# domkirke/acids_transforms

Hardware: AMD Instinct MI355X
Metric: spectrogram frames/sec (fwd+invert), n_fft=1024 hop=256 (higher is better)
Workload: dtype f32; 1 GPU; configs[1]: batch=1024 clips/GPU x 4 s mono 44.1 kHz, STFT fwd + Magnitude(mel=128, log1p, unipolar) [one fused kernel] + ISTFT invert, fp32; n_fft=1024, hop=256, frames_per_clip=690, clips_per_gpu=1024

## Files before the change

### acids_transforms_amd/csrc/fft512.h

```cpp
#pragma once
#include <hip/hip_runtime.h>
#include <stdint.h>

#include "fastmath.h"
#include "inv1024_pairs.h"

namespace at_hip {

#ifndef AT_WAVE_PRIORITY
#define AT_WAVE_PRIORITY 1
#endif
template <int LEVEL>
__device__ __forceinline__ void wave_priority() {
#if AT_WAVE_PRIORITY
  __builtin_amdgcn_s_setprio(LEVEL);
#endif
}

constexpr int kFftLdsFloat2PerWave = 568;

constexpr int kTwiddleCount = 22 * 64;
constexpr int kTileCtrSlots = 4096;

__device__ __forceinline__ float2 cadd(float2 a, float2 b) { return make_float2(a.x + b.x, a.y + b.y); }

typedef float v2f __attribute__((ext_vector_type(2)));

__device__ __forceinline__ v2f to_v(float2 a) { return (v2f){a.x, a.y}; }
// ... 110 lines not shown
  __device__ __forceinline__ v2f getr(int m) const { return tr[m]; }
  __device__ __forceinline__ v2f getr_self() const { return tr_self; }
};

template <bool INV>
struct LdsTwiddles {
  const float2* tab;
  int lane;
  __device__ __forceinline__ v2f get1(int k) const { return lds_read_single(reinterpret_cast<const v2f*>(tab) + k * 64 + lane); }
  __device__ __forceinline__ v2f get2(int k) const { return lds_read_single(reinterpret_cast<const v2f*>(tab) + (7 + k) * 64 + lane); }
  __device__ __forceinline__ v2f getr(int m) const { return lds_read_single(reinterpret_cast<const v2f*>(tab) + (14 + m) * 64 + lane); }
  __device__ __forceinline__ v2f getr_self() const { return lds_read_single(reinterpret_cast<const v2f*>(tab) + (14 + inv1024::kSelfPairedRow) * 64); }
};
struct HybridTwiddles {
  v2f t1[7];
  v2f t2[7];
  const float2* tab;
  int col;
  __device__ __forceinline__ v2f get1(int k) const { return t1[k]; }
  __device__ __forceinline__ v2f get2(int k) const { return t2[k]; }
  __device__ __forceinline__ v2f getr(int m) const { return lds_read_single(reinterpret_cast<const v2f*>(tab) + (14 + m) * 64 + col); }
};

template <bool INV>
__device__ __forceinline__ float2 twiddle_for_lds(const float2* __restrict__ tab, int i) {
  const float2 a = tab[i];
  return (!INV && i >= 14 * 64) ? make_float2(0.5f * a.x, 0.5f * a.y) : a;
}

template <bool INV>
__device__ __forceinline__ void load_twiddles(Twiddles& tw, const float2* __restrict__ tab, int lane) {
#pragma unroll
  for (int k = 0; k < 7; ++k) {
    tw.t1[k] = to_v(tab[k * 64 + lane]);
    tw.t2[k] = to_v(tab[(7 + k) * 64 + lane]);
  }
#pragma unroll
  for (int m = 0; m < 8; ++m) tw.tr[m] = to_v(twiddle_for_lds<INV>(tab, (14 + m) * 64 + lane));
  if (INV) {
    const float2 w = tab[(14 + inv1024::kSelfPairedRow) * 64];
    tw.tr_self = (v2f){__int_as_float(__builtin_amdgcn_readfirstlane(__float_as_int(w.x))),
                       __int_as_float(__builtin_amdgcn_readfirstlane(__float_as_int(w.y)))};
  }
}

#ifndef AT_XCHG1_SWAP
// ... 17 lines not shown
        const auto sw = __builtin_amdgcn_permlane16_swap(__float_as_uint(v[k][c]), __float_as_uint(v[k + 2][c]), false, false);
        v[k][c] = __uint_as_float(sw[0]);
        v[k + 2][c] = __uint_as_float(sw[1]);
      }
#pragma unroll
  for (int k = 0; k < 8; k += 2)
#pragma unroll
    for (int c = 0; c < 2; ++c) {
      const int a = __float_as_int(v[k][c]), b = __float_as_int(v[k + 1][c]);
      const int a2 = __builtin_amdgcn_update_dpp(a, b, 0x128, 0xf, 0xc, false);
      const int b2 = __builtin_amdgcn_update_dpp(b, a, 0x128, 0xf, 0x3, false);
      v[k][c] = __int_as_float(a2);
      v[k + 1][c] = __int_as_float(b2);
    }
}

template <bool INV, typename TW>
__device__ __forceinline__ void fft512(v2f (&v)[8], const TW& tw, float2* lds_f2, int lane, int out_lane = -1) {
  if (out_lane < 0) out_lane = lane;
  v2f* lds = reinterpret_cast<v2f*>(lds_f2);
  const int lo = lane & 7, hi = lane >> 3;
  radix8<INV>(v);
#pragma unroll
  for (int k = 1; k < 8; ++k) v[k] = twiddle<INV>(v[k], tw.get1(k - 1));
  if constexpr (AT_XCHG1_SWAP == 2 || (AT_XCHG1_SWAP == 1 && !INV)) {
    xchg1_registers(v);
  } else {
#pragma unroll
    for (int k = 0; k < 8; ++k) lds[hi * 72 + lo + 8 * k] = v[k];
    wave_lds_sync();
#pragma unroll
    for (int k = 0; k < 8; ++k) v[k] = lds_read_single(lds + k * 72 + lane);
    wave_lds_sync();
  }
  radix8<INV>(v);
#pragma unroll
  for (int k = 1; k < 8; ++k) v[k] = twiddle<INV>(v[k], tw.get2(k - 1));
#pragma unroll
  for (int k = 0; k < 8; ++k) lds[lo * 66 + hi + 8 * k] = v[k];
  wave_lds_sync();
#pragma unroll
  for (int k = 0; k < 8; ++k) v[k] = lds_read_single(lds + k * 66 + out_lane);
  wave_lds_sync();
  radix8<INV>(v);
}
constexpr bool fft512_exchanges_cover(int lo_slot, int hi_slot) {
  for (int s = lo_slot; s <= hi_slot; ++s) {
    bool hit = false;
    for (int a = 0; a < 8 && !hit; ++a) {
      if (s >= a * 72 && s < a * 72 + 64) hit = true;
      if (s >= a * 66 && s < a * 66 + 64) hit = true;
    }
    if (!hit) return false;
  }
  return true;
}
static_assert(AT_XCHG1_SWAP || (fft512_exchanges_cover(256, 319) && 320 <= kFftLdsFloat2PerWave),
              "the fixed-length mel epilogue reads absrow[513..639] uncleared: both exchanges must rewrite float2 slots 256..319");

template <bool INV, typename TW>
// ... 53 lines not shown
template <int Q, int WS>
__device__ __forceinline__ void irfft_presplit(const v2f (&x)[Q], float nyq_re, int lane, const v2f* w, v2f (&z)[Q]) {
  v2f v[Q], pm[Q];
#pragma unroll
  for (int m = 0; m < Q; ++m) v[m] = x[m];
  if (lane == 0) v[0].y = 0.0f;
  mirror_regs<Q>(v, pm, lane);
  if (lane == 0) pm[0] = (v2f){nyq_re, 0.0f};
#pragma unroll
  for (int m = 0; m < Q; ++m) {
    const v2f e = add_conj(v[m], pm[m]);
    const v2f d = cmul_conj_v(sub_conj(v[m], pm[m]), w[WS * m]);
    z[m] = add_pi(e, d);
  }
}

template <typename TW>
__device__ __forceinline__ void rfft_merge(v2f (&v)[8], const TW& tw, int lane, float2& nyq) {
  const v2f hh = {0.5f, 0.5f};
  v2f p[8];
  mirror_regs<8>(v, p, lane);
  nyq = make_float2(v[0].x - v[0].y, 0.0f);
#pragma unroll
  for (int m = 0; m < 8; ++m) {
    const v2f e = add_conj(v[m], p[m]);
    const v2f d = sub_conj(v[m], p[m]);
    const v2f wd = cmul_v(d, tw.getr(m));
    v[m] = scale_add_mi(e, hh, wd);
  }
}
template <typename TW>
__device__ __forceinline__ void rfft_merge_rot(v2f (&v)[8], const TW& tw, int lane, int rot, int col, float2& nyq) {
  const v2f hh = {0.5f, 0.5f};
  v2f p[8];
  mirror_regs_rot<8>(v, p, lane, rot, col);
  nyq = make_float2(v[0].x - v[0].y, 0.0f);
#pragma unroll
  for (int m = 0; m < 8; ++m) {
    const v2f e = add_conj(v[m], p[m]);
    const v2f d = sub_conj(v[m], p[m]);
    const v2f wd = cmul_v(d, tw.getr(m));
    v[m] = scale_add_mi(e, hh, wd);
  }
}
template <typename TW>
__device__ __forceinline__ void rfft_merge(float2 (&f)[8], const TW& tw, int lane, float2& nyq) {
  v2f v[8];
#pragma unroll
  for (int m = 0; m < 8; ++m) v[m] = to_v(f[m]);
  rfft_merge(v, tw, lane, nyq);
#pragma unroll
  for (int m = 0; m < 8; ++m) f[m] = to_f2(v[m]);
}

template <typename TW>
__device__ __forceinline__ void irfft_split(v2f (&v)[8], const TW& tw, int lane, v2f x256) {
  if (lane == 0) {
    v[0].y = 0.0f;
    v[7].y = 0.0f;
  }
#pragma unroll
  for (int m = 0; m < inv1024::kPairs; ++m) {
    const int n = inv1024::partner_reg(m);
    const v2f e = add_conj(v[m], v[n]);
    const v2f d = cmul_conj_v(sub_conj(v[m], v[n]), tw.getr(m));
// ... 63 lines not shown
```

### acids_transforms_amd/csrc/stft1024.hip

```cpp
#include <hip/hip_runtime.h>
#include "fastmath.h"
#include <type_traits>
#include <stdint.h>
#include <stdlib.h>
#include <stdio.h>
#include <string.h>
#include <atomic>

#include "band_bank.h"
#include "fft512.h"
#include "fwd1024_forms.h"
#include "run_plan.h"
#include "stft_launch.h"
#include "variants.h"

#ifndef AT_ISTFT_NT
#define AT_ISTFT_NT 1
#endif
#ifndef AT_ISTFT_NTLOAD
#define AT_ISTFT_NTLOAD 1
#endif

namespace at_hip {

constexpr int N = 1024;
constexpr int F = 513;
constexpr int WAVES_PER_BLOCK = 4;

struct FwdParams {
  const float* x;
  const float* window;
  const float2* tw;
  float2* out;
  float* phase;
  long long B, L, clip_stride, T;
  long long total_frames;
  long long frames_per_block;
  int hop;
  int center;
};

__device__ __forceinline__ void load_frame(const FwdParams& p, long long f, int lane, float2 (&v)[8]) {
  const long long b = f / p.T;
// ... 97 lines not shown
__device__ __forceinline__ float2 load_pair(const float* clip, long long L, long long i0, bool interior, bool aligned,
                                            int lane_off) {
  if (interior) {
    if (aligned) return reinterpret_cast<const float2*>(clip + i0)[lane_off >> 1];
    return make_float2(clip[i0 + lane_off], clip[i0 + lane_off + 1]);
  }
  return make_float2(clip[reflect_index(i0 + lane_off, L)], clip[reflect_index(i0 + lane_off + 1, L)]);
}


__device__ __forceinline__ float fwd_contrast(float v, int mode, float eps) { return band_contrast_fast(v, mode, eps); }

template <class Form>
__global__ __launch_bounds__(64 * Form::waves, fwd1024::waves_per_simd<Form>()) void stft1024_h256_fwd_kernel(FwdRunParams p) {
  constexpr bool WRITE_PHASE = Form::write_phase, TWLDS = Form::lds_twiddles, POLAR = Form::polar;
  constexpr bool AL = Form::aligned_stores, NT = Form::nontemporal, FP2 = Form::fixed_power2, PW = Form::persistent;
  constexpr int MEL = Form::mel, FWD_WAVES = Form::waves, CMBUF = Form::window_passes, HS = Form::hop_slots;
  constexpr int SP = Form::hoisted_passes, FQ0 = Form::fixed_quads0, FQ1 = Form::fixed_quads1, FC = Form::fixed_contrast;
  constexpr int HYB = Form::register_tables, FNP = Form::packed_passes;
  constexpr fqp_t FQP = Form::packed_quads;
  constexpr int H = 128 * HS;
  constexpr int kNP = FQP ? FNP : 1;
  constexpr int kPkStride = (kNP + 3) / 4 * 4;
  constexpr int kTabTw = TWLDS ? kTwiddleCount : 0;
  constexpr int kFeatCarry = FQP ? 128 : 0;
  constexpr int kWaveLds = kFftLdsFloat2PerWave + kFeatCarry;
  __shared__ float2 lds_all[FWD_WAVES * kWaveLds + kTabTw + 512];
  extern __shared__ float4 band_lds[];
  const int lane = threadIdx.x & 63;
  const int wave = __builtin_amdgcn_readfirstlane(threadIdx.x >> 6);
  float2* lds = lds_all + wave * kWaveLds + kFeatCarry;
  float2* tab = lds_all + FWD_WAVES * kWaveLds;
  float2 raw_first[8];
  auto load_first_frame = [&](const long long run, float2 (&raw)[8]) {
    const long long b = run / p.runs_per_clip;
    if (b >= p.B) return;
    const long long t0 = (run - b * p.runs_per_clip) * p.frames_per_run;
    if (t0 >= p.T) return;
    const float* clip = p.x + b * p.clip_stride;
    const bool clip_aligned = ((((uintptr_t)clip) & 7) == 0);
    const long long s0 = t0 * (128 * HS) - 512;
#pragma unroll
    for (int m = 0; m < 8; ++m) {
      const long long i0 = s0 + 128 * m;
      raw[m] = load_pair(clip, p.L, i0, i0 >= 0 && i0 + 128 <= p.L, clip_aligned, 2 * lane);
    }
  };
  if constexpr (!PW) load_first_frame((long long)blockIdx.x * FWD_WAVES + wave, raw_first);
  if (TWLDS)
    for (int i = threadIdx.x; i < kTwiddleCount; i += 64 * FWD_WAVES) tab[i] = twiddle_for_lds<false>(p.tw, i);
  for (int i = threadIdx.x; i < 512; i += 64 * FWD_WAVES)
    tab[kTabTw + i] = reinterpret_cast<const float2*>(p.window)[i];
  float* wlds = reinterpret_cast<float*>(band_lds);
  int* lane_tab = nullptr;
  if (MEL != 0) {
    int table_floats = 0;
    for (int q = 0; q < p.bank.n_passes; ++q) table_floats += 64 * p.bank.pass_len[q];
    for (int i = threadIdx.x; i < table_floats; i += 64 * FWD_WAVES) wlds[i] = p.bank.weights[i];
    lane_tab = reinterpret_cast<int*>(wlds + table_floats);
    for (int i = threadIdx.x; i < 64 * p.bank.n_passes; i += 64 * FWD_WAVES) {
      lane_tab[i] = p.bank.lane_start[i];
      lane_tab[64 * p.bank.n_passes + i] = p.bank.lane_filter[i];
    }
    if constexpr (FQP != 0) {
      int* pk_tab = lane_tab + 2 * 64 * p.bank.n_passes;
      for (int i = threadIdx.x; i < 64 * kNP; i += 64 * FWD_WAVES) {
        const int q = i >> 6, l = i & 63;
        const int f = p.bank.lane_filter[i];
        pk_tab[l * kPkStride + q] = (p.bank.lane_start[i] * 4) | ((f >= 0 ? f * 4 : 0xfff) << 12);
      }
    }
  }
  __shared__ unsigned s_tile[2];
  if (PW && threadIdx.x == 0) s_tile[0] = atomicAdd(p.tile_ctr, 1u);
#if AT_XCHG1_SWAP
  if (MEL != 0) {
    reinterpret_cast<float*>(lds)[512 + lane] = 0.0f;
    reinterpret_cast<float*>(lds)[576 + lane] = 0.0f;
  }
#endif
  __syncthreads();

  int sp_f[SP > 0 ? SP : 1], sp_start[SP > 0 ? SP : 1], sp_quads[SP > 0 ? SP : 1];
  if constexpr (SP > 0) {
#pragma unroll
    for (int q = 0; q < SP; ++q) {
      sp_f[q] = lane_tab[(SP + q) * 64 + lane];
      sp_start[q] = lane_tab[q * 64 + lane];
      sp_quads[q] = p.bank.pass_len[q] >> 2;
    }
  }
  Twiddles tw_regs;
  if (!TWLDS) load_twiddles<false>(tw_regs, p.tw, lane);
  const LdsTwiddles<false> tw_lds = {tab, lane};
  HybridTwiddles tw_hyb;
  if constexpr (TWLDS && (HYB & 1)) {
#pragma unroll
    for (int k = 0; k < 7; ++k) {
      tw_hyb.t1[k] = to_v(p.tw[k * 64 + lane]);
      tw_hyb.t2[k] = to_v(p.tw[(7 + k) * 64 + lane]);
    }
    tw_hyb.tab = tab;
    tw_hyb.col = lane;
  }
  const float2* win = tab + kTabTw;
  v2f win_regs[8];
  if constexpr ((HYB & 2) != 0) {
#pragma unroll
    for (int m = 0; m < 8; ++m) win_regs[m] = to_v(reinterpret_cast<const float2*>(p.window)[lane + 64 * m]);
  }

  const long long L = p.L;
  const int lane2 = 2 * lane;

  auto do_run = [&](const long long run, const bool preloaded) {
  const long long b = run / p.runs_per_clip;
  if (b >= p.B) return;
  const long long r = run - b * p.runs_per_clip;
// ... 47 lines not shown
  };
  long long t_cur = t0;
  float cm[CMBUF ? CMBUF : 1][8];
  int cm_held[CMBUF ? CMBUF : 1];
#pragma unroll
  for (int q = 0; q < (CMBUF ? CMBUF : 1); ++q) {
    cm_held[q] = 0;
#pragma unroll
    for (int k = 0; k < 8; ++k) cm[q][k] = 0.f;
  }
  float mel_off = 0.f, mel_inv = 1.f;
  if (MEL != 0 && p.offset) {
    mel_off = *p.offset;
    mel_inv = 1.0f / *p.scale;
  }

  float2 nyq_pending = make_float2(0.f, 0.f);
  float2* nyq_dst = nullptr;
  auto flush_nyquist = [&]() {
    if (nyq_dst != nullptr && lane == 0) *nyq_dst = nyq_pending;
    if (WRITE_PHASE && nyq_dst != nullptr && lane == 0)
      p.phase[(nyq_dst - p.out)] = fast_atan2f(nyq_pending.y, nyq_pending.x);
  };
  auto frame_body = [&](const float2 (&fresh)[HS]) {
    wave_priority<3>();
    float2 v[8];
#pragma unroll
    for (int m = 0; m < 8; ++m) {
      const v2f w = (HYB & 2) ? win_regs[m] : lds_read_single(reinterpret_cast<const v2f*>(win) + lane + 64 * m);
      v[m] = make_float2(raw[m].x * w.x, raw[m].y * w.y);
    }
#pragma unroll
    for (int m = 0; m < 8 - HS; ++m) raw[m] = raw[m + HS];
#pragma unroll
    for (int k = 0; k < HS; ++k) raw[8 - HS + k] = fresh[k];
    float2 nyq;
    const int col = AL ? ((lane - rot) & 63) : lane;
    {
      v2f z[8];
#pragma unroll
      for (int m = 0; m < 8; ++m) z[m] = to_v(v[m]);
      if constexpr (AL && (HYB & 1)) {
        fft512<false>(z, tw_hyb, lds, lane, col);
        tw_hyb.col = col;
        rfft_merge_rot(z, tw_hyb, lane, rot, col, nyq);
      } else if constexpr (AL) {
        fft512<false>(z, tw_lds, lds, lane, col);
        const LdsTwiddles<false> tw_col = {tab, col};
        rfft_merge_rot(z, tw_col, lane, rot, col, nyq);
      } else if constexpr (TWLDS && (HYB & 1)) {
        fft512<false>(z, tw_hyb, lds, lane);
        rfft_merge(z, tw_hyb, lane, nyq);
      } else if (TWLDS) {
        fft512<false>(z, tw_lds, lds, lane);
        rfft_merge(z, tw_lds, lane, nyq);
      } else {
        fft512<false>(z, tw_regs, lds, lane);
        rfft_merge(z, tw_regs, lane, nyq);
      }
#pragma unroll
      for (int m = 0; m < 8; ++m) v[m] = to_f2(z[m]);
      if constexpr (AL) {
        wave_priority<1>();
        const bool lo = lane < rot;
        const v2f s0 = lo ? carry : z[0];
        if (head) {
          if (!lo) put(sp, s0);
          head = false;
        } else {
          put(sp, s0);
        }
// ... 205 lines not shown
        one_pass(0, std::integral_constant<int, 0>());
        if constexpr (CMBUF >= 2) one_pass(1, std::integral_constant<int, 1>());
      } else if constexpr (SP >= 1) {
        one_pass(0, std::integral_constant<int, -1>());
        if constexpr (SP >= 2) one_pass(1, std::integral_constant<int, -1>());
      } else {
        for (int q = 0; q < p.bank.n_passes; ++q) one_pass(q, std::integral_constant<int, -1>());
      }
      wave_lds_sync();
      frow += feat_ld;
      ++t_cur;
    }
    nyq_pending = nyq;
    nyq_dst = (MEL != 2 && !AL) ? row + 512 : nullptr;
    row += F;
  };

  long long t = t0;
  long long t_fast_end = (L >= 512) ? (L - 512) / H : 0;
  if (t_fast_end > t1) t_fast_end = t1;
  if (!clip_aligned) t_fast_end = t0;
  if (t < t_fast_end) {
    const float2* nsrc = reinterpret_cast<const float2*>(clip + t * H + 512) + lane;
    for (; t < t_fast_end; ++t) {
      flush_nyquist();
      float2 fresh[HS];
#pragma unroll
      for (int k = 0; k < HS; ++k) fresh[k] = nsrc[64 * k];
      nsrc += H / 2;
      frame_body(fresh);
    }
  }
  for (; t < t1; ++t) {
    flush_nyquist();
    float2 fresh[HS];
#pragma unroll
    for (int k = 0; k < HS; ++k) fresh[k] = make_float2(0.f, 0.f);
    if (t + 1 < t1) {
#pragma unroll
      for (int k = 0; k < HS; ++k) {
        const long long i0 = t * H + 512 + 128 * k;
        fresh[k] = load_pair(clip, L, i0, i0 >= 0 && i0 + 128 <= L, clip_aligned, lane2);
      }
    }
    frame_body(fresh);
  }
  flush_nyquist();
  if constexpr (AL) {
    if (lane < rot) put(sp, carry);
  }
  if constexpr (FQP != 0) {
    wave_lds_sync();
    const float* fbuf = reinterpret_cast<const float*>(lds) - 2 * kFeatCarry;
    const float4 v = reinterpret_cast<const float4*>(fbuf)[lane];
    const float vv[4] = {v.x, v.y, v.z, v.w};
#pragma unroll
    for (int c = 0; c < 4; ++c)
      if (4 * lane + c < fc && 4 * lane + c >= fhead) fdst[4 * lane + c] = vv[c];
    wave_lds_sync();
  }
  };

  if constexpr (!PW) {
    do_run((long long)blockIdx.x * FWD_WAVES + wave, true);
  } else {
    for (int it = 0;; ++it) {
      const unsigned tile = __builtin_amdgcn_readfirstlane(s_tile[it & 1]);
      if (tile >= p.n_tiles) break;
// ... 123 lines not shown
  x256 = gl_update(q.rmid, q.tmid, q.amid, mom);
}

template <int IN_MODE>
__device__ __forceinline__ void load_spectrum(const InvParams& p, long long f, int lane, float2 (&v)[8], float2& x256) {
  RawFrame<IN_MODE> q;
  load_raw(p, f, lane, q);
  raw_to_spectrum(q, v, x256);
}

__device__ __forceinline__ float2 scaled_window(const float* window, int i) {
  const float2 w = reinterpret_cast<const float2*>(window)[i];
  return make_float2(w.x * (1.0f / 1024.0f), w.y * (1.0f / 1024.0f));
}

template <typename TW>
__device__ __forceinline__ void synth_frame_nowin(const float2 (&v)[8], float2 x256, const TW& tw, float2* lds, int lane,
                                                  v2f (&z)[8]) {
#pragma unroll
  for (int m = 0; m < 8; ++m) z[m] = to_v(v[m]);
  irfft_split(z, tw, lane, to_v(x256));
  fft512<true>(z, tw, lds, lane);
}
__device__ __forceinline__ v2f ola_window(const float2* win, int lane, int m) {
  return lds_read_single(reinterpret_cast<const v2f*>(win) + lane + 64 * m);
}

template <typename TW>
__device__ __forceinline__ void synth_frame(float2 (&v)[8], float2 x256, const TW& tw, const float2* win,
                                            float2* lds, int lane) {
  v2f z[8];
#pragma unroll
  for (int m = 0; m < 8; ++m) z[m] = to_v(v[m]);
  irfft_split(z, tw, lane, to_v(x256));
  fft512<true>(z, tw, lds, lane);
#pragma unroll
  for (int m = 0; m < 8; ++m) {
    const v2f w = lds_read_single(reinterpret_cast<const v2f*>(win) + lane + 64 * m);
    v[m] = to_f2(z[m] * w);
  }
}

template <int IN_MODE, int DEPTH, bool TWLDS, int HS = 2>
__global__ __launch_bounds__(64 * WAVES_PER_BLOCK, IN_MODE == IN_GL ? 2 : (TWLDS ? 5 : 4) - DEPTH) void istft1024_ola_kernel(InvParams p) {
  constexpr int R = 8 / HS;
  constexpr int C = 4 / HS;
  constexpr int H = 128 * HS;
  constexpr int kFull = (1 << R) - 1;
  __shared__ float2 lds_all[WAVES_PER_BLOCK * kFftLdsFloat2PerWave + 512 + (TWLDS ? kTwiddleCount : 0)];
  const int lane = threadIdx.x & 63;
  const int wave = __builtin_amdgcn_readfirstlane(threadIdx.x >> 6);
  float2* lds = lds_all + wave * kFftLdsFloat2PerWave;
  float2* win = lds_all + WAVES_PER_BLOCK * kFftLdsFloat2PerWave;
  float2* twtab = win + 512;
  for (int i = threadIdx.x; i < 512; i += 64 * WAVES_PER_BLOCK) win[i] = scaled_window(p.window, i);
  if (TWLDS)
    for (int i = threadIdx.x; i < kTwiddleCount; i += 64 * WAVES_PER_BLOCK) twtab[i] = p.tw[i];
  __syncthreads();

  const long long run = (long long)blockIdx.x * WAVES_PER_BLOCK + wave;
  const long long b = run / p.runs_per_clip;
  if (b >= p.B) return;
  const long long r = run - b * p.runs_per_clip;
  const long long nslots = p.T - 1;
  const long long j0 = r * p.slots_per_run;
  long long j1 = j0 + p.slots_per_run;
  if (j1 > nslots) j1 = nslots;
  if (j0 >= j1) return;

  Twiddles tw_regs;
  if (!TWLDS) load_twiddles<true>(tw_regs, p.tw, lane);
  const LdsTwiddles<true> tw_lds = {twtab, lane};
  auto synth = [&](const float2 (&v)[8], float2 x256, v2f (&z)[8]) {
    if (TWLDS) synth_frame_nowin(v, x256, tw_lds, lds, lane, z);
    else synth_frame_nowin(v, x256, tw_regs, lds, lane, z);
  };

  v2f acc[8];
#pragma unroll
  for (int m = 0; m < 8; ++m) acc[m] = (v2f){0.f, 0.f};

  const long long fbase = b * p.T;
  float* yclip = p.y + b * (H * nslots);
  long long t = (j0 + C - (R - 1) > 0) ? j0 + C - (R - 1) : 0;
  const long long t_last = j1 - 1 + C;
  const long long t_have = (t_last < p.T - 1) ? t_last : p.T - 1;

  RawFrame<IN_MODE> q0 = {}, q1 = {};
  if (t <= t_have) load_raw(p, fbase + t, lane, q0);
  if (t + 1 <= t_have) load_raw(p, fbase + t + 1, lane, q1);

  auto consume = [&](const RawFrame<IN_MODE>& q) {
    float2 v[8];
    float2 x256;
    if constexpr (IN_MODE == IN_GL) raw_to_spectrum(q, v, x256, p.gl_mom);
    else raw_to_spectrum(q, v, x256);
    v2f z[8];
    synth(v, x256, z);
#pragma unroll
    for (int m = 0; m < 8; ++m) acc[m] = __builtin_elementwise_fma(z[m], ola_window(win, lane, m), acc[m]);
  };
  auto put_y = [&](float2* dst, float2 val) {
#if AT_ISTFT_NT
    __builtin_nontemporal_store((v2f){val.x, val.y}, reinterpret_cast<v2f*>(dst));
#else
    *dst = val;
#endif
  };
  static_assert(sizeof(v2f) == sizeof(float2), "");
  auto emit = [&](long long j, const float2* env) {
    float2* dst = reinterpret_cast<float2*>(yclip + j * H);
#pragma unroll
    for (int k = 0; k < HS; ++k) {
      const float2 e = env[lane + 64 * k];
      put_y(dst + lane + 64 * k, make_float2(acc[k].x / e.x, acc[k].y / e.y));
    }
  };
  float2 rcp[HS];
  auto emit_fast = [&](long long j) {
    float2* dst = reinterpret_cast<float2*>(yclip + j * H);
#pragma unroll
    for (int k = 0; k < HS; ++k) put_y(dst + lane + 64 * k, make_float2(acc[k].x * rcp[k].x, acc[k].y * rcp[k].y));
  };
// ... 26 lines not shown
        const long long tt = t - (R - 1) + q;
        if (tt >= 0 && tt < p.T) mask |= 1 << q;
      }
      if (mask == kFull) emit_fast(j);
      else emit(j, reinterpret_cast<const float2*>(p.env + mask * H));
    }
    advance();
    ++t;
  };

  long long fast_begin = j0 + C > R - 1 ? j0 + C : R - 1;
  long long fast_end = (j1 - 1 + C < t_have - 2) ? j1 - 1 + C : t_have - 2;
  while (t < fast_begin && t <= t_last) generic_step();
  if (t <= fast_end) {
    if (DEPTH == 2) {
      auto fast_step = [&](RawFrame<IN_MODE>& q) {
        const RawFrame<IN_MODE> cur = q;
        load_raw(p, fbase + t + 2, lane, q);
        consume(cur);
        emit_fast(t - C);
        advance();
        ++t;
      };
      while (t + 1 <= fast_end) {
        fast_step(q0);
        fast_step(q1);
      }
    } else {
      q1 = {};
      for (; t <= fast_end; ++t) {
        const RawFrame<IN_MODE> cur = q0;
        load_raw(p, fbase + t + 1, lane, q0);
        consume(cur);
        emit_fast(t - C);
        advance();
      }
      q1 = {};
      if (t + 1 <= t_have) load_raw(p, fbase + t + 1, lane, q1);
    }
  }
  while (t <= t_last) generic_step();
}

template <int IN_MODE, int NW, int OCC>
__global__ __launch_bounds__(64 * NW, OCC) void istft1024_tile_kernel(InvParams p) {
  constexpr int HS = 2, R = 4, H = 256;
  constexpr int kFull = (1 << R) - 1;
  static_assert(IN_MODE != IN_GL, "the Griffin-Lim form keeps the long-run kernel");
  __shared__ float2 lds_all[NW * kFftLdsFloat2PerWave + 512];
  __shared__ float4 park_all[NW * 6 * 64];
  const int lane = threadIdx.x & 63;
  const int wave = __builtin_amdgcn_readfirstlane(threadIdx.x >> 6);
  float2* lds = lds_all + wave * kFftLdsFloat2PerWave;
  float2* win = lds_all + NW * kFftLdsFloat2PerWave;

  const long long tile = blockIdx.x;
  const long long b = tile / p.runs_per_clip;
  const long long k = tile - b * p.runs_per_clip;
  const long long n = p.slots_per_run;
  const long long T = p.T;
  const long long tile0 = k * p.frames_per_block;
  long long tile1 = tile0 + p.frames_per_block;
  if (tile1 > T) tile1 = T;
  auto share = [&](int w, long long& a, long long& e) {
    a = tile0 + w * n;
    if (a > tile1) a = tile1;
    e = (w == NW - 1) ? tile1 : a + n;
    if (e > tile1) e = tile1;
  };
  long long ta, tb;
  share(wave, ta, tb);
  bool self_cool = true;
  if (wave < NW - 1) {
    long long a2, e2;
    share(wave + 1, a2, e2);
    self_cool = e2 - a2 < 3;
  }
  long long t_stop = (self_cool && tb > ta) ? tb + 3 : tb;
  if (t_stop > T) t_stop = T;
  const bool parks = wave > 0 && ta > 0;
  const long long pe0 = ta == 0 ? 2 : ta + 3;
  const long long pe1 = tb + 3;

  const long long fbase = b * T;
  float* yclip = p.y + b * (H * (T - 1));
  long long t = ta;
  RawFrame<IN_MODE> q0 = {}, q1 = {};
  if (t < t_stop) load_raw(p, fbase + t, lane, q0);
  if (t + 1 < t_stop) load_raw(p, fbase + t + 1, lane, q1);

  for (int i = threadIdx.x; i < 512; i += 64 * NW) win[i] = scaled_window(p.window, i);
  Twiddles tw;
  load_twiddles<true>(tw, p.tw, lane);
  __syncthreads();

  v2f acc[8];
#pragma unroll
  for (int m = 0; m < 8; ++m) acc[m] = (v2f){0.f, 0.f};
  auto consume = [&](const RawFrame<IN_MODE>& q, v2f (&z)[8]) {
    float2 v[8];
    float2 x256;
    raw_to_spectrum(q, v, x256);
    synth_frame_nowin(v, x256, tw, lds, lane, z);
#pragma unroll
    for (int m = 0; m < 8; ++m) acc[m] = __builtin_elementwise_fma(z[m], ola_window(win, lane, m), acc[m]);
  };
  auto put_y = [&](float2* dst, float2 val) {
    __builtin_nontemporal_store((v2f){val.x, val.y}, reinterpret_cast<v2f*>(dst));
  };
  float2 rcp[HS];
  {
    const float2* env_full = reinterpret_cast<const float2*>(p.env + kFull * H);
#pragma unroll
    for (int kk = 0; kk < HS; ++kk) {
      const float2 e = env_full[lane + 64 * kk];
      rcp[kk] = make_float2(1.0f / e.x, 1.0f / e.y);
    }
  }
  auto emit_regs = [&](long long hp, v2f a0, v2f a1) {
    float2* dst = reinterpret_cast<float2*>(yclip + (hp - 2) * H);
    if (hp >= 3 && hp < T) {
      put_y(dst + lane, make_float2(a0.x * rcp[0].x, a0.y * rcp[0].y));
      put_y(dst + lane + 64, make_float2(a1.x * rcp[1].x, a1.y * rcp[1].y));
    } else {
      int mask = 0;
#pragma unroll
      for (int q = 0; q < R; ++q) {
        const long long tt = hp - (R - 1) + q;
// ... 27 lines not shown
    }
    if (t >= pe0 && t < pe1) emit_regs(t, acc[0], acc[1]);
    advance();
    ++t;
  };

  long long fast_begin = ta + 3 > pe0 ? ta + 3 : pe0;
  if (fast_begin < 3) fast_begin = 3;
  long long fast_end = tb - 1;
  if (fast_end > t_stop - 3) fast_end = t_stop - 3;
  while (t < fast_begin && t < tb) generic_step();
  if (t <= fast_end) {
    auto fast_step = [&](RawFrame<IN_MODE>& q) {
      const RawFrame<IN_MODE> cur = q;
      load_raw(p, fbase + t + 2, lane, q);
      v2f v[8];
      consume(cur, v);
      float2* dst = reinterpret_cast<float2*>(yclip + (t - 2) * H);
      put_y(dst + lane, make_float2(acc[0].x * rcp[0].x, acc[0].y * rcp[0].y));
      put_y(dst + lane + 64, make_float2(acc[1].x * rcp[1].x, acc[1].y * rcp[1].y));
      advance();
      ++t;
    };
    while (t + 1 <= fast_end) {
      fast_step(q0);
      fast_step(q1);
    }
  }
  while (t < tb) generic_step();
  __syncthreads();
  if (self_cool) {
    while (t < t_stop) generic_step();
    if (t_stop == T && T >= pe0 && T < pe1 && t == T) emit_regs(T, acc[0], acc[1]);
  } else if (tb > ta) {
    const float4* nx = park_all + (wave + 1) * 6 * 64 + lane;
    auto add4 = [&](int hop, int s, const float4 pc) {
      acc[2 * hop] = __builtin_elementwise_fma((v2f){pc.x, pc.y}, ola_window(win, lane, 2 * s), acc[2 * hop]);
      acc[2 * hop + 1] = __builtin_elementwise_fma((v2f){pc.z, pc.w}, ola_window(win, lane, 2 * s + 1), acc[2 * hop + 1]);
    };
    add4(0, 0, nx[0 * 64]);
    add4(1, 1, nx[1 * 64]);
    add4(1, 0, nx[3 * 64]);
    add4(2, 2, nx[2 * 64]);
    add4(2, 1, nx[4 * 64]);
    add4(2, 0, nx[5 * 64]);
#pragma unroll
    for (int s = 0; s < 3; ++s)
      if (tb + s >= pe0) emit_regs(tb + s, acc[2 * s], acc[2 * s + 1]);
  }
}

template <int IN_MODE>
__global__ __launch_bounds__(64 * WAVES_PER_BLOCK) void irfft1024_frames_kernel(InvParams p) {
  __shared__ float2 lds_all[WAVES_PER_BLOCK * kFftLdsFloat2PerWave + 512];
  const int lane = threadIdx.x & 63;
  const int wave = threadIdx.x >> 6;
  float2* lds = lds_all + wave * kFftLdsFloat2PerWave;
  float2* win = lds_all + WAVES_PER_BLOCK * kFftLdsFloat2PerWave;
  for (int i = threadIdx.x; i < 512; i += 64 * WAVES_PER_BLOCK) win[i] = scaled_window(p.window, i);
  __syncthreads();
  Twiddles tw;
// ... 238 lines not shown
```

Measured before the change: 469.5 million frames/s.

## Interleave LDS twiddle/window rows into pairs and rotate OLA accumulators

Stores LDS twiddle and window tables as interleaved row pairs so each lane fetches two rows with one 16-byte LDS read instead of two 8-byte reads. It also adds a four-phase unrolled inverse loop that rotates accumulator indices instead of shifting registers each frame. The forward rename path is off by default. The trade-offs are extra padding slots, 16-byte LDS alignment, and larger unrolled code that may raise register pressure.

```diff
diff --git a/acids_transforms_amd/csrc/fft512.h b/acids_transforms_amd/csrc/fft512.h
--- a/acids_transforms_amd/csrc/fft512.h
+++ b/acids_transforms_amd/csrc/fft512.h
@@ -4,6 +4,11 @@
 
 #include "fastmath.h"
 #include "inv1024_pairs.h"
+#include "lds_row_pairs.h"
+
+#ifndef AT_LDS_ROW_PAIRS
+#define AT_LDS_ROW_PAIRS 1
+#endif
 
 namespace at_hip {
 
@@ -160,6 +165,51 @@
   __device__ __forceinline__ v2f getr(int m) const { return lds_read_single(reinterpret_cast<const v2f*>(tab) + (14 + m) * 64 + col); }
 };
 
+typedef float v4f __attribute__((ext_vector_type(4)));
+__device__ __forceinline__ void lds_read_row_pair(const float2* tab, int pair, int col, v2f& a, v2f& b) {
+  const v4f q = lds_read_single(reinterpret_cast<const v4f*>(tab) + row_pairs::element(pair, col));
+  a = (v2f){q.x, q.y};
+  b = (v2f){q.z, q.w};
+}
+template <bool INV>
+struct PairedLdsTwiddles {
+  const float2* tab;
+  int lane;
+  int pass_lane;
+};
+struct PairedHybridTwiddles {
+  v2f t1[7];
+  v2f t2[7];
+  const float2* tab;
+  int col;
+  __device__ __forceinline__ v2f get1(int k) const { return t1[k]; }
+  __device__ __forceinline__ v2f get2(int k) const { return t2[k]; }
+};
+template <typename TW> __device__ __forceinline__ void tw_pair1(const TW& tw, int j, v2f& a, v2f& b) {
+  a = tw.get1(2 * j);
+  b = (2 * j + 1 < 7) ? tw.get1(2 * j + 1) : a;
+}
+template <typename TW> __device__ __forceinline__ void tw_pair2(const TW& tw, int j, v2f& a, v2f& b) {
+  a = tw.get2(2 * j);
+  b = (2 * j + 1 < 7) ? tw.get2(2 * j + 1) : a;
+}
+template <typename TW> __device__ __forceinline__ void tw_pairr(const TW& tw, int j, v2f& a, v2f& b) {
+  a = tw.getr(2 * j);
+  b = tw.getr(2 * j + 1);
+}
+template <bool INV> __device__ __forceinline__ void tw_pair1(const PairedLdsTwiddles<INV>& tw, int j, v2f& a, v2f& b) {
+  lds_read_row_pair(tw.tab, row_pairs::kPass1Pair0 + j, tw.pass_lane, a, b);
+}
+template <bool INV> __device__ __forceinline__ void tw_pair2(const PairedLdsTwiddles<INV>& tw, int j, v2f& a, v2f& b) {
+  lds_read_row_pair(tw.tab, row_pairs::kPass2Pair0 + j, tw.pass_lane, a, b);
+}
+template <bool INV> __device__ __forceinline__ void tw_pairr(const PairedLdsTwiddles<INV>& tw, int j, v2f& a, v2f& b) {
+  lds_read_row_pair(tw.tab, row_pairs::kMergePair0 + j, tw.lane, a, b);
+}
+__device__ __forceinline__ void tw_pairr(const PairedHybridTwiddles& tw, int j, v2f& a, v2f& b) {
+  lds_read_row_pair(tw.tab, row_pairs::kMergePair0 + j, tw.col, a, b);
+}
+
 template <bool INV>
 __device__ __forceinline__ float2 twiddle_for_lds(const float2* __restrict__ tab, int i) {
   const float2 a = tab[i];
@@ -223,7 +273,12 @@
   const int lo = lane & 7, hi = lane >> 3;
   radix8<INV>(v);
 #pragma unroll
-  for (int k = 1; k < 8; ++k) v[k] = twiddle<INV>(v[k], tw.get1(k - 1));
+  for (int j = 0; j < 4; ++j) {
+    v2f a, b;
+    tw_pair1(tw, j, a, b);
+    v[2 * j + 1] = twiddle<INV>(v[2 * j + 1], a);
+    if (j < 3) v[2 * j + 2] = twiddle<INV>(v[2 * j + 2], b);
+  }
   if constexpr (AT_XCHG1_SWAP == 2 || (AT_XCHG1_SWAP == 1 && !INV)) {
     xchg1_registers(v);
   } else {
@@ -236,7 +291,12 @@
   }
   radix8<INV>(v);
 #pragma unroll
-  for (int k = 1; k < 8; ++k) v[k] = twiddle<INV>(v[k], tw.get2(k - 1));
+  for (int j = 0; j < 4; ++j) {
+    v2f a, b;
+    tw_pair2(tw, j, a, b);
+    v[2 * j + 1] = twiddle<INV>(v[2 * j + 1], a);
+    if (j < 3) v[2 * j + 2] = twiddle<INV>(v[2 * j + 2], b);
+  }
 #pragma unroll
   for (int k = 0; k < 8; ++k) lds[lo * 66 + hi + 8 * k] = v[k];
   wave_lds_sync();
@@ -336,11 +396,16 @@
   mirror_regs<8>(v, p, lane);
   nyq = make_float2(v[0].x - v[0].y, 0.0f);
 #pragma unroll
-  for (int m = 0; m < 8; ++m) {
-    const v2f e = add_conj(v[m], p[m]);
-    const v2f d = sub_conj(v[m], p[m]);
-    const v2f wd = cmul_v(d, tw.getr(m));
-    v[m] = scale_add_mi(e, hh, wd);
+  for (int j = 0; j < 4; ++j) {
+    v2f w[2];
+    tw_pairr(tw, j, w[0], w[1]);
+#pragma unroll
+    for (int m = 2 * j; m < 2 * j + 2; ++m) {
+      const v2f e = add_conj(v[m], p[m]);
+      const v2f d = sub_conj(v[m], p[m]);
+      const v2f wd = cmul_v(d, w[m & 1]);
+      v[m] = scale_add_mi(e, hh, wd);
+    }
   }
 }
 template <typename TW>
@@ -350,11 +415,16 @@
   mirror_regs_rot<8>(v, p, lane, rot, col);
   nyq = make_float2(v[0].x - v[0].y, 0.0f);
 #pragma unroll
-  for (int m = 0; m < 8; ++m) {
-    const v2f e = add_conj(v[m], p[m]);
-    const v2f d = sub_conj(v[m], p[m]);
-    const v2f wd = cmul_v(d, tw.getr(m));
-    v[m] = scale_add_mi(e, hh, wd);
+  for (int j = 0; j < 4; ++j) {
+    v2f w[2];
+    tw_pairr(tw, j, w[0], w[1]);
+#pragma unroll
+    for (int m = 2 * j; m < 2 * j + 2; ++m) {
+      const v2f e = add_conj(v[m], p[m]);
+      const v2f d = sub_conj(v[m], p[m]);
+      const v2f wd = cmul_v(d, w[m & 1]);
+      v[m] = scale_add_mi(e, hh, wd);
+    }
   }
 }
 template <typename TW>
diff --git a/acids_transforms_amd/csrc/lds_row_pairs.h b/acids_transforms_amd/csrc/lds_row_pairs.h
--- /dev/null
+++ b/acids_transforms_amd/csrc/lds_row_pairs.h
@@ -0,0 +1,54 @@
+#pragma once
+
+namespace at_hip {
+namespace row_pairs {
+
+constexpr int kLanes = 64;
+constexpr int kPass1Rows = 7, kPass2Rows = 7, kMergeRows = 8, kWindowRows = 8;
+constexpr int pairs_of(int rows) { return (rows + 1) / 2; }
+constexpr int kPass1Pair0 = 0;
+constexpr int kPass2Pair0 = kPass1Pair0 + pairs_of(kPass1Rows);
+constexpr int kMergePair0 = kPass2Pair0 + pairs_of(kPass2Rows);
+constexpr int kTwiddlePairs = kMergePair0 + pairs_of(kMergeRows);
+constexpr int kWindowPairs = pairs_of(kWindowRows);
+constexpr int kTwiddleSlots = 2 * kLanes * kTwiddlePairs;
+constexpr int kWindowSlots = 2 * kLanes * kWindowPairs;
+
+constexpr int element(int pair, int col) { return pair * kLanes + col; }
+constexpr int half_of(int row) { return row & 1; }
+constexpr int slot(int pair0, int row, int col) { return 2 * element(pair0 + row / 2, col) + half_of(row); }
+constexpr int rotated_col(int lane, int rot) { return (lane - rot) & (kLanes - 1); }
+constexpr int read_element(int pair0, int j, int lane, int rot) { return element(pair0 + j, rotated_col(lane, rot)); }
+constexpr int bank_group(int elem) { return elem % 16; }
+
+constexpr int twiddle_slot(int i) {
+  const int row = i / kLanes, lane = i % kLanes;
+  return row < kPass1Rows ? slot(kPass1Pair0, row, lane)
+       : row < kPass1Rows + kPass2Rows ? slot(kPass2Pair0, row - kPass1Rows, lane)
+                                       : slot(kMergePair0, row - kPass1Rows - kPass2Rows, lane);
+}
+constexpr int twiddle_pad_slot(int p) {
+  return p < kLanes ? slot(kPass1Pair0, kPass1Rows, p) : slot(kPass2Pair0, kPass2Rows, p - kLanes);
+}
+constexpr int window_slot(int i) { return slot(0, i / kLanes, i % kLanes); }
+
+constexpr bool slots_are_a_permutation() {
+  bool seen[kTwiddleSlots] = {};
+  for (int i = 0; i < 22 * kLanes; ++i) {
+    const int s = twiddle_slot(i);
+    if (s < 0 || s >= kTwiddleSlots || seen[s]) return false;
+    seen[s] = true;
+  }
+  for (int p = 0; p < 2 * kLanes; ++p) {
+    const int s = twiddle_pad_slot(p);
+    if (s < 0 || s >= kTwiddleSlots || seen[s]) return false;
+    seen[s] = true;
+  }
+  for (int s = 0; s < kTwiddleSlots; ++s)
+    if (!seen[s]) return false;
+  return true;
+}
+static_assert(slots_are_a_permutation(), "every slot of the paired twiddle table is one table entry or one padding entry");
+
+}
+}
diff --git a/acids_transforms_amd/csrc/stft1024.hip b/acids_transforms_amd/csrc/stft1024.hip
--- a/acids_transforms_amd/csrc/stft1024.hip
+++ b/acids_transforms_amd/csrc/stft1024.hip
@@ -19,6 +19,12 @@
 #endif
 #ifndef AT_ISTFT_NTLOAD
 #define AT_ISTFT_NTLOAD 1
+#endif
+#ifndef AT_FWD_RENAME
+#define AT_FWD_RENAME 0
+#endif
+#ifndef AT_INV_RENAME
+#define AT_INV_RENAME 1
 #endif
 
 namespace at_hip {
@@ -162,10 +168,12 @@
   constexpr int H = 128 * HS;
   constexpr int kNP = FQP ? FNP : 1;
   constexpr int kPkStride = (kNP + 3) / 4 * 4;
-  constexpr int kTabTw = TWLDS ? kTwiddleCount : 0;
+  constexpr bool PAIRS = AT_LDS_ROW_PAIRS != 0;
+  constexpr int kTabTw = TWLDS ? (PAIRS ? row_pairs::kTwiddleSlots : kTwiddleCount) : 0;
   constexpr int kFeatCarry = FQP ? 128 : 0;
   constexpr int kWaveLds = kFftLdsFloat2PerWave + kFeatCarry;
-  __shared__ float2 lds_all[FWD_WAVES * kWaveLds + kTabTw + 512];
+  static_assert((FWD_WAVES * kWaveLds) % 2 == 0 && kTabTw % 2 == 0, "the tables are read 16 bytes at a time");
+  __shared__ __attribute__((aligned(16))) float2 lds_all[FWD_WAVES * kWaveLds + kTabTw + 512];
   extern __shared__ float4 band_lds[];
   const int lane = threadIdx.x & 63;
   const int wave = __builtin_amdgcn_readfirstlane(threadIdx.x >> 6);
@@ -187,10 +195,13 @@
     }
   };
   if constexpr (!PW) load_first_frame((long long)blockIdx.x * FWD_WAVES + wave, raw_first);
-  if (TWLDS)
-    for (int i = threadIdx.x; i < kTwiddleCount; i += 64 * FWD_WAVES) tab[i] = twiddle_for_lds<false>(p.tw, i);
+  if (TWLDS) {
+    for (int i = threadIdx.x; i < kTwiddleCount; i += 64 * FWD_WAVES)
+      tab[PAIRS ? row_pairs::twiddle_slot(i) : i] = twiddle_for_lds<false>(p.tw, i);
+    if (PAIRS && threadIdx.x < 128) tab[row_pairs::twiddle_pad_slot(threadIdx.x)] = make_float2(0.f, 0.f);
+  }
   for (int i = threadIdx.x; i < 512; i += 64 * FWD_WAVES)
-    tab[kTabTw + i] = reinterpret_cast<const float2*>(p.window)[i];
+    tab[kTabTw + (PAIRS ? row_pairs::window_slot(i) : i)] = reinterpret_cast<const float2*>(p.window)[i];
   float* wlds = reinterpret_cast<float*>(band_lds);
   int* lane_tab = nullptr;
   if (MEL != 0) {
@@ -232,8 +243,17 @@
   }
   Twiddles tw_regs;
   if (!TWLDS) load_twiddles<false>(tw_regs, p.tw, lane);
-  const LdsTwiddles<false> tw_lds = {tab, lane};
-  HybridTwiddles tw_hyb;
+  using LdsTw = std::conditional_t<PAIRS, PairedLdsTwiddles<false>, LdsTwiddles<false>>;
+  using HybTw = std::conditional_t<PAIRS, PairedHybridTwiddles, HybridTwiddles>;
+  auto lds_tw = [&](int col) {
+#if AT_LDS_ROW_PAIRS
+    return LdsTw{tab, col, lane};
+#else
+    return LdsTw{tab, col};
+#endif
+  };
+  const LdsTw tw_lds = lds_tw(lane);
+  HybTw tw_hyb;
   if constexpr (TWLDS && (HYB & 1)) {
 #pragma unroll
     for (int k = 0; k < 7; ++k) {
@@ -327,18 +347,39 @@
     if (WRITE_PHASE && nyq_dst != nullptr && lane == 0)
       p.phase[(nyq_dst - p.out)] = fast_atan2f(nyq_pending.y, nyq_pending.x);
   };
-  auto frame_body = [&](const float2 (&fresh)[HS]) {
+  auto frame_body = [&](auto phase, auto&& fetch) {
+    constexpr int PH = decltype(phase)::value;
+    constexpr int S0 = PH < 0 ? 0 : (HS * PH) & 7;
+    float2 fresh[HS];
+    if constexpr (PH < 0) fetch(fresh);
     wave_priority<3>();
     float2 v[8];
 #pragma unroll
-    for (int m = 0; m < 8; ++m) {
-      const v2f w = (HYB & 2) ? win_regs[m] : lds_read_single(reinterpret_cast<const v2f*>(win) + lane + 64 * m);
-      v[m] = make_float2(raw[m].x * w.x, raw[m].y * w.y);
-    }
-#pragma unroll
-    for (int m = 0; m < 8 - HS; ++m) raw[m] = raw[m + HS];
-#pragma unroll
-    for (int k = 0; k < HS; ++k) raw[8 - HS + k] = fresh[k];
+    for (int j = 0; j < 4; ++j) {
+      v2f w[2];
+      if constexpr ((HYB & 2) != 0) {
+        w[0] = win_regs[2 * j];
+        w[1] = win_regs[2 * j + 1];
+      } else if constexpr (PAIRS) {
+        lds_read_row_pair(win, j, lane, w[0], w[1]);
+      } else {
+        w[0] = lds_read_single(reinterpret_cast<const v2f*>(win) + lane + 64 * (2 * j));
+        w[1] = lds_read_single(reinterpret_cast<const v2f*>(win) + lane + 64 * (2 * j + 1));
+      }
+#pragma unroll
+      for (int m = 2 * j; m < 2 * j + 2; ++m)
+        v[m] = make_float2(raw[(m + S0) & 7].x * w[m & 1].x, raw[(m + S0) & 7].y * w[m & 1].y);
+    }
+    if constexpr (PH < 0) {
+#pragma unroll
+      for (int m = 0; m < 8 - HS; ++m) raw[m] = raw[m + HS];
+#pragma unroll
+      for (int k = 0; k < HS; ++k) raw[8 - HS + k] = fresh[k];
+    } else {
+      fetch(fresh);
+#pragma unroll
+      for (int k = 0; k < HS; ++k) raw[(S0 + k) & 7] = fresh[k];
+    }
     float2 nyq;
     const int col = AL ? ((lane - rot) & 63) : lane;
     {
@@ -351,7 +392,7 @@
         rfft_merge_rot(z, tw_hyb, lane, rot, col, nyq);
       } else if constexpr (AL) {
         fft512<false>(z, tw_lds, lds, lane, col);
-        const LdsTwiddles<false> tw_col = {tab, col};
+        const LdsTw tw_col = lds_tw(col);
         rfft_merge_rot(z, tw_col, lane, rot, col, nyq);
       } else if constexpr (TWLDS && (HYB & 1)) {
         fft512<false>(z, tw_hyb, lds, lane);
@@ -603,28 +644,43 @@
   if (!clip_aligned) t_fast_end = t0;
   if (t < t_fast_end) {
     const float2* nsrc = reinterpret_cast<const float2*>(clip + t * H + 512) + lane;
+    auto fetch_next = [&](float2 (&fresh)[HS]) {
+#pragma unroll
+      for (int k = 0; k < HS; ++k) fresh[k] = nsrc[64 * k];
+      nsrc += H / 2;
+    };
+    constexpr bool TRIPS = AT_FWD_RENAME != 0 && AL && HS == 2;
+    if constexpr (TRIPS) {
+      constexpr int TRIP = 8 / HS;
+      for (; t + TRIP <= t_fast_end; t += TRIP) {
+        flush_nyquist();
+        frame_body(std::integral_constant<int, 0>(), fetch_next);
+        flush_nyquist();
+        frame_body(std::integral_constant<int, 1>(), fetch_next);
+        flush_nyquist();
+        frame_body(std::integral_constant<int, 2>(), fetch_next);
+        flush_nyquist();
+        frame_body(std::integral_constant<int, 3>(), fetch_next);
+      }
+    }
     for (; t < t_fast_end; ++t) {
       flush_nyquist();
-      float2 fresh[HS];
-#pragma unroll
-      for (int k = 0; k < HS; ++k) fresh[k] = nsrc[64 * k];
-      nsrc += H / 2;
-      frame_body(fresh);
+      frame_body(std::integral_constant<int, -1>(), fetch_next);
     }
   }
   for (; t < t1; ++t) {
     flush_nyquist();
-    float2 fresh[HS];
-#pragma unroll
-    for (int k = 0; k < HS; ++k) fresh[k] = make_float2(0.f, 0.f);
-    if (t + 1 < t1) {
-#pragma unroll
-      for (int k = 0; k < HS; ++k) {
-        const long long i0 = t * H + 512 + 128 * k;
-        fresh[k] = load_pair(clip, L, i0, i0 >= 0 && i0 + 128 <= L, clip_aligned, lane2);
-      }
-    }
-    frame_body(fresh);
+    frame_body(std::integral_constant<int, -1>(), [&](float2 (&fresh)[HS]) {
+#pragma unroll
+      for (int k = 0; k < HS; ++k) fresh[k] = make_float2(0.f, 0.f);
+      if (t + 1 < t1) {
+#pragma unroll
+        for (int k = 0; k < HS; ++k) {
+          const long long i0 = t * H + 512 + 128 * k;
+          fresh[k] = load_pair(clip, L, i0, i0 >= 0 && i0 + 128 <= L, clip_aligned, lane2);
+        }
+      }
+    });
   }
   flush_nyquist();
   if constexpr (AL) {
@@ -794,8 +850,25 @@
   irfft_split(z, tw, lane, to_v(x256));
   fft512<true>(z, tw, lds, lane);
 }
-__device__ __forceinline__ v2f ola_window(const float2* win, int lane, int m) {
-  return lds_read_single(reinterpret_cast<const v2f*>(win) + lane + 64 * m);
+__device__ __forceinline__ void ola_window_pair(const float2* win, int lane, int j, v2f& a, v2f& b) {
+#if AT_LDS_ROW_PAIRS
+  lds_read_row_pair(win, j, lane, a, b);
+#else
+  a = lds_read_single(reinterpret_cast<const v2f*>(win) + lane + 64 * (2 * j));
+  b = lds_read_single(reinterpret_cast<const v2f*>(win) + lane + 64 * (2 * j + 1));
+#endif
+}
+__device__ __forceinline__ int ola_window_slot(int i) { return AT_LDS_ROW_PAIRS ? row_pairs::window_slot(i) : i; }
+template <int S0>
+__device__ __forceinline__ void ola_accumulate(const v2f (&z)[8], const float2* win, int lane, v2f (&acc)[8]) {
+#pragma unroll
+  for (int j = 0; j < 4; ++j) {
+    v2f w[2];
+    ola_window_pair(win, lane, j, w[0], w[1]);
+#pragma unroll
+    for (int m = 2 * j; m < 2 * j + 2; ++m)
+      acc[(m + S0) & 7] = __builtin_elementwise_fma(z[m], w[m & 1], acc[(m + S0) & 7]);
+  }
 }
 
 template <typename TW>
@@ -819,13 +892,13 @@
   constexpr int C = 4 / HS;
   constexpr int H = 128 * HS;
   constexpr int kFull = (1 << R) - 1;
-  __shared__ float2 lds_all[WAVES_PER_BLOCK * kFftLdsFloat2PerWave + 512 + (TWLDS ? kTwiddleCount : 0)];
+  __shared__ __attribute__((aligned(16))) float2 lds_all[WAVES_PER_BLOCK * kFftLdsFloat2PerWave + 512 + (TWLDS ? kTwiddleCount : 0)];
   const int lane = threadIdx.x & 63;
   const int wave = __builtin_amdgcn_readfirstlane(threadIdx.x >> 6);
   float2* lds = lds_all + wave * kFftLdsFloat2PerWave;
   float2* win = lds_all + WAVES_PER_BLOCK * kFftLdsFloat2PerWave;
   float2* twtab = win + 512;
-  for (int i = threadIdx.x; i < 512; i += 64 * WAVES_PER_BLOCK) win[i] = scaled_window(p.window, i);
+  for (int i = threadIdx.x; i < 512; i += 64 * WAVES_PER_BLOCK) win[ola_window_slot(i)] = scaled_window(p.window, i);
   if (TWLDS)
     for (int i = threadIdx.x; i < kTwiddleCount; i += 64 * WAVES_PER_BLOCK) twtab[i] = p.tw[i];
   __syncthreads();
@@ -869,8 +942,7 @@
     else raw_to_spectrum(q, v, x256);
     v2f z[8];
     synth(v, x256, z);
-#pragma unroll
-    for (int m = 0; m < 8; ++m) acc[m] = __builtin_elementwise_fma(z[m], ola_window(win, lane, m), acc[m]);
+    ola_accumulate<0>(z, win, lane, acc);
   };
   auto put_y = [&](float2* dst, float2 val) {
 #if AT_ISTFT_NT
@@ -943,6 +1015,33 @@
         advance();
         ++t;
       };
+      if constexpr (AT_INV_RENAME != 0 && HS == 2 && DEPTH == 2 && !TWLDS && IN_MODE != IN_GL) {
+        auto trip_step = [&](auto phase, RawFrame<IN_MODE>& q) {
+          constexpr int S0 = (2 * decltype(phase)::value) & 7;
+          float2 v[8];
+          float2 x256;
+          raw_to_spectrum(q, v, x256);
+          v2f z[8];
+#pragma unroll
+          for (int m = 0; m < 8; ++m) z[m] = to_v(v[m]);
+          irfft_split(z, tw_regs, lane, to_v(x256));
+          load_raw(p, fbase + t + 2, lane, q);
+          fft512<true>(z, tw_regs, lds, lane);
+          ola_accumulate<S0>(z, win, lane, acc);
+          float2* dst = reinterpret_cast<float2*>(yclip + (t - C) * H);
+          put_y(dst + lane, make_float2(acc[S0].x * rcp[0].x, acc[S0].y * rcp[0].y));
+          put_y(dst + lane + 64, make_float2(acc[S0 + 1].x * rcp[1].x, acc[S0 + 1].y * rcp[1].y));
+          acc[S0] = (v2f){0.f, 0.f};
+          acc[S0 + 1] = (v2f){0.f, 0.f};
+          ++t;
+        };
+        while (t + 3 <= fast_end) {
+          trip_step(std::integral_constant<int, 0>(), q0);
+          trip_step(std::integral_constant<int, 1>(), q1);
+          trip_step(std::integral_constant<int, 2>(), q0);
+          trip_step(std::integral_constant<int, 3>(), q1);
+        }
+      }
       while (t + 1 <= fast_end) {
         fast_step(q0);
         fast_step(q1);
@@ -968,7 +1067,7 @@
   constexpr int HS = 2, R = 4, H = 256;
   constexpr int kFull = (1 << R) - 1;
   static_assert(IN_MODE != IN_GL, "the Griffin-Lim form keeps the long-run kernel");
-  __shared__ float2 lds_all[NW * kFftLdsFloat2PerWave + 512];
+  __shared__ __attribute__((aligned(16))) float2 lds_all[NW * kFftLdsFloat2PerWave + 512];
   __shared__ float4 park_all[NW * 6 * 64];
   const int lane = threadIdx.x & 63;
   const int wave = __builtin_amdgcn_readfirstlane(threadIdx.x >> 6);
@@ -1010,7 +1109,7 @@
   if (t < t_stop) load_raw(p, fbase + t, lane, q0);
   if (t + 1 < t_stop) load_raw(p, fbase + t + 1, lane, q1);
 
-  for (int i = threadIdx.x; i < 512; i += 64 * NW) win[i] = scaled_window(p.window, i);
+  for (int i = threadIdx.x; i < 512; i += 64 * NW) win[ola_window_slot(i)] = scaled_window(p.window, i);
   Twiddles tw;
   load_twiddles<true>(tw, p.tw, lane);
   __syncthreads();
@@ -1023,8 +1122,7 @@
     float2 x256;
     raw_to_spectrum(q, v, x256);
     synth_frame_nowin(v, x256, tw, lds, lane, z);
-#pragma unroll
-    for (int m = 0; m < 8; ++m) acc[m] = __builtin_elementwise_fma(z[m], ola_window(win, lane, m), acc[m]);
+    ola_accumulate<0>(z, win, lane, acc);
   };
   auto put_y = [&](float2* dst, float2 val) {
     __builtin_nontemporal_store((v2f){val.x, val.y}, reinterpret_cast<v2f*>(dst));
@@ -1098,6 +1196,33 @@
       advance();
       ++t;
     };
+    if constexpr (AT_INV_RENAME != 0) {
+      auto trip_step = [&](auto phase, RawFrame<IN_MODE>& q) {
+        constexpr int S0 = (2 * decltype(phase)::value) & 7;
+        float2 v[8];
+        float2 x256;
+        raw_to_spectrum(q, v, x256);
+        v2f z[8];
+#pragma unroll
+        for (int m = 0; m < 8; ++m) z[m] = to_v(v[m]);
+        irfft_split(z, tw, lane, to_v(x256));
+        load_raw(p, fbase + t + 2, lane, q);
+        fft512<true>(z, tw, lds, lane);
+        ola_accumulate<S0>(z, win, lane, acc);
+        float2* dst = reinterpret_cast<float2*>(yclip + (t - 2) * H);
+        put_y(dst + lane, make_float2(acc[S0].x * rcp[0].x, acc[S0].y * rcp[0].y));
+        put_y(dst + lane + 64, make_float2(acc[S0 + 1].x * rcp[1].x, acc[S0 + 1].y * rcp[1].y));
+        acc[S0] = (v2f){0.f, 0.f};
+        acc[S0 + 1] = (v2f){0.f, 0.f};
+        ++t;
+      };
+      while (t + 3 <= fast_end) {
+        trip_step(std::integral_constant<int, 0>(), q0);
+        trip_step(std::integral_constant<int, 1>(), q1);
+        trip_step(std::integral_constant<int, 2>(), q0);
+        trip_step(std::integral_constant<int, 3>(), q1);
+      }
+    }
     while (t + 1 <= fast_end) {
       fast_step(q0);
       fast_step(q1);
@@ -1111,8 +1236,10 @@
   } else if (tb > ta) {
     const float4* nx = park_all + (wave + 1) * 6 * 64 + lane;
     auto add4 = [&](int hop, int s, const float4 pc) {
-      acc[2 * hop] = __builtin_elementwise_fma((v2f){pc.x, pc.y}, ola_window(win, lane, 2 * s), acc[2 * hop]);
-      acc[2 * hop + 1] = __builtin_elementwise_fma((v2f){pc.z, pc.w}, ola_window(win, lane, 2 * s + 1), acc[2 * hop + 1]);
+      v2f w0, w1;
+      ola_window_pair(win, lane, s, w0, w1);
+      acc[2 * hop] = __builtin_elementwise_fma((v2f){pc.x, pc.y}, w0, acc[2 * hop]);
+      acc[2 * hop + 1] = __builtin_elementwise_fma((v2f){pc.z, pc.w}, w1, acc[2 * hop + 1]);
     };
     add4(0, 0, nx[0 * 64]);
     add4(1, 1, nx[1 * 64]);
```

Result: no change. 472.6 million frames/s, median of 2 (+0.7%).
